# 3DOM-FBK/deep-image-matching

Hardware: NVIDIA H100
Metric: image-pairs/sec (SuperPoint+LightGlue, 1024x1024, 2048 kpts) (higher is better)
Workload: dtype f16 hi/lo split x3 MMA, f32 accumulate (fp32-class)

## Files before the change

### deep-image-matching_b200/csrc/attention.cuh

```cuda
#pragma once
#include "common.cuh"
#include "sm90.cuh"

namespace {

constexpr int kAttnBlk = 64;
constexpr int kAttnTile = 128;
constexpr int kAttnThreads = 9 * 32;

template <int HD, bool SPLIT>
struct AttnGeom {
  static constexpr int kPl = SPLIT ? 2 : 1;
  static constexpr int kAtoms = HD / 64;
  static constexpr int kAtomQ = kAttnTile * 128, kQB = kAtoms * kAtomQ;
  static constexpr int kAtomK = kAttnBlk * 128, kKB = kAtoms * kAtomK;
  static constexpr int kVB = HD * 128;
  static constexpr int kSmem = kPl * (kQB + 2 * (kKB + kVB)) + 256 + 1024;
};

template <int HD, bool SPLIT, class Out>
__device__ __forceinline__ void attn_tile(const CUtensorMap* tmQh, const CUtensorMap* tmQl, const CUtensorMap* tmKh,
                                          const CUtensorMap* tmKl, const CUtensorMap* tmVh, const CUtensorMap* tmVl, int qrow, int krow,
                                          int vrow, int nq, int nk, float scale, float lazy, const Out& out) {
  using namespace sm90;
  using G = AttnGeom<HD, SPLIT>;
  extern __shared__ uint8_t sm_attn_raw[];
  uint8_t* smem = sm_attn_raw + ((1024u - (smem_u32(sm_attn_raw) & 1023u)) & 1023u);
  uint8_t* sQ = smem;
  uint8_t* sK = sQ + G::kPl * G::kQB;
  uint8_t* sV = sK + 2 * G::kPl * G::kKB;
  uint64_t* bars = reinterpret_cast<uint64_t*>(sV + 2 * G::kPl * G::kVB);
  uint64_t *bQ = bars, *kFull = bars + 1, *kEmpty = bars + 3, *vFull = bars + 5, *vEmpty = bars + 7;
  const int tid = threadIdx.x, warp = tid >> 5, lane = tid & 31;
  if (tid == 0) {
    mbar_init(bQ, 1);
    for (int i = 0; i < 2; ++i) {
      mbar_init(&kFull[i], 1);
      mbar_init(&kEmpty[i], 8);
      mbar_init(&vFull[i], 1);
      mbar_init(&vEmpty[i], 8);
    }
    fence_barrier_init();
  }
  __syncthreads();
  const int nblk = (nk + kAttnBlk - 1) / kAttnBlk;

  if (warp == 8) {
    if (nblk > 0 && elect_one()) {
      mbar_expect_tx(bQ, G::kPl * G::kQB);
      for (int at = 0; at < G::kAtoms; ++at) {
        tma_load_2d(sQ + at * G::kAtomQ, tmQh, bQ, at * 64, qrow);
        if (SPLIT) tma_load_2d(sQ + G::kQB + at * G::kAtomQ, tmQl, bQ, at * 64, qrow);
      }
    }
    __syncwarp();
    for (int j = 0; j < nblk; ++j) {
      const int s = j & 1;
      const uint32_t ph = (j >> 1) & 1;
      mbar_wait(&kEmpty[s], ph ^ 1);
      if (elect_one()) {
        mbar_expect_tx(&kFull[s], G::kPl * G::kKB);
        for (int at = 0; at < G::kAtoms; ++at) {
          tma_load_2d(sK + s * G::kPl * G::kKB + at * G::kAtomK, tmKh, &kFull[s], at * 64, krow + j * kAttnBlk);
          if (SPLIT) tma_load_2d(sK + s * G::kPl * G::kKB + G::kKB + at * G::kAtomK, tmKl, &kFull[s], at * 64, krow + j * kAttnBlk);
        }
      }
      __syncwarp();
      mbar_wait(&vEmpty[s], ph ^ 1);
      if (elect_one()) {
        mbar_expect_tx(&vFull[s], G::kPl * G::kVB);
        tma_load_2d(sV + s * G::kPl * G::kVB, tmVh, &vFull[s], j * kAttnBlk, vrow);
        if (SPLIT) tma_load_2d(sV + s * G::kPl * G::kVB + G::kVB, tmVl, &vFull[s], j * kAttnBlk, vrow);
      }
      __syncwarp();
    }
    return;
  }
  const int wg = warp >> 2, w4 = warp & 3;
  const int r0 = 64 * wg + 16 * w4 + (lane >> 2);
  const uint32_t q_wg = smem_u32(sQ) + wg * 64 * 128;
  float o[HD / 2];
#pragma unroll
  for (int i = 0; i < HD / 2; ++i) o[i] = 0.f;
  float m_run[2] = {-INFINITY, -INFINITY}, l_run[2] = {0.f, 0.f};
  const float c2 = scale * 1.4426950408889634f;
  if (nblk > 0) mbar_wait(bQ, 0);
  for (int j = 0; j < nblk; ++j) {
    const int s = j & 1;
    const uint32_t ph = (j >> 1) & 1;
    float sc[kAttnBlk / 2];
    mbar_wait(&kFull[s], ph);
    {
      const uint32_t kb = smem_u32(sK + s * G::kPl * G::kKB);
      wgmma_fence();
#pragma unroll
      for (int kk = 0; kk < 4 * G::kAtoms; ++kk) {
        const uint64_t qh = sdesc_advance_k(make_sdesc_sw128(q_wg + (kk >> 2) * G::kAtomQ), kk & 3);
        const uint64_t kh = sdesc_advance_k(make_sdesc_sw128(kb + (kk >> 2) * G::kAtomK), kk & 3);
        Wgmma<kAttnBlk>::ss(sc, qh, kh, kk != 0);
        if (SPLIT) {
          const uint64_t ql = sdesc_advance_k(make_sdesc_sw128(q_wg + G::kQB + (kk >> 2) * G::kAtomQ), kk & 3);
          const uint64_t kl = sdesc_advance_k(make_sdesc_sw128(kb + G::kKB + (kk >> 2) * G::kAtomK), kk & 3);
          Wgmma<kAttnBlk>::ss(sc, qh, kl, 1);
          Wgmma<kAttnBlk>::ss(sc, ql, kh, 1);
        }
      }
      wgmma_commit();
      wgmma_wait<0>();
      wgmma_fence_regs(sc);
    }
    if (lane == 0) mbar_arrive(&kEmpty[s]);
    const int key0 = j * kAttnBlk + 2 * (lane & 3);
    if (j * kAttnBlk + kAttnBlk > nk) {
#pragma unroll
      for (int i = 0; i < kAttnBlk / 8; ++i)
#pragma unroll
        for (int e = 0; e < 4; ++e)
          if (key0 + 8 * i + (e & 1) >= nk) sc[4 * i + e] = -INFINITY;
    }
    float alpha[2], mc[2];
#pragma unroll
    for (int h = 0; h < 2; ++h) {
      float mx = sc[2 * h];
#pragma unroll
      for (int i = 0; i < kAttnBlk / 8; ++i) mx = fmaxf(mx, fmaxf(sc[4 * i + 2 * h], sc[4 * i + 2 * h + 1]));
      mx = fmaxf(mx, __shfl_xor_sync(0xffffffffu, mx, 1));
      mx = fmaxf(mx, __shfl_xor_sync(0xffffffffu, mx, 2));
      const float m_blk = fmaxf(m_run[h], mx);
      const bool grow = (m_blk - m_run[h]) * c2 > lazy;
      const float m_new = grow ? m_blk : m_run[h];
      alpha[h] = grow ? fast_exp2((m_run[h] - m_new) * c2) : 1.f;
      mc[h] = m_new * c2;
      m_run[h] = m_new;
    }
    float ps[2] = {0.f, 0.f};
#pragma unroll
    for (int i = 0; i < kAttnBlk / 8; ++i)
#pragma unroll
      for (int e = 0; e < 4; ++e) {
        sc[4 * i + e] = fast_exp2(fmaf(sc[4 * i + e], c2, -mc[e >> 1]));
        ps[e >> 1] += sc[4 * i + e];
      }
#pragma unroll
    for (int h = 0; h < 2; ++h) l_run[h] = l_run[h] * alpha[h] + ps[h];
#pragma unroll
    for (int i = 0; i < HD / 8; ++i) {
      o[4 * i] *= alpha[0], o[4 * i + 1] *= alpha[0];
      o[4 * i + 2] *= alpha[1], o[4 * i + 3] *= alpha[1];
    }
    uint32_t ph_[kAttnBlk / 4], pl_[kAttnBlk / 4];
#pragma unroll
    for (int c = 0; c < kAttnBlk / 4; ++c) {
      __half2 h2, l2;
      split2_f32(sc[2 * c], sc[2 * c + 1], h2, l2);
      ph_[c] = *reinterpret_cast<uint32_t*>(&h2);
      pl_[c] = *reinterpret_cast<uint32_t*>(&l2);
    }
    mbar_wait(&vFull[s], ph);
    {
      const uint32_t vb = smem_u32(sV + s * G::kPl * G::kVB);
      const uint64_t v_h = make_sdesc_sw128(vb), v_l = make_sdesc_sw128(vb + G::kVB);
      wgmma_fence();
#pragma unroll
      for (int kk = 0; kk < kAttnBlk / 16; ++kk) {
        const uint32_t ah[4] = {ph_[4 * kk], ph_[4 * kk + 1], ph_[4 * kk + 2], ph_[4 * kk + 3]};
        Wgmma<HD>::rs(o, ah, sdesc_advance_k(v_h, kk), 1);
        if (SPLIT) {
          const uint32_t al[4] = {pl_[4 * kk], pl_[4 * kk + 1], pl_[4 * kk + 2], pl_[4 * kk + 3]};
          Wgmma<HD>::rs(o, ah, sdesc_advance_k(v_l, kk), 1);
          Wgmma<HD>::rs(o, al, sdesc_advance_k(v_h, kk), 1);
        }
      }
      wgmma_commit();
      wgmma_wait<0>();
      wgmma_fence_regs(o);
    }
    if (lane == 0) mbar_arrive(&vEmpty[s]);
  }
  float inv[2];
#pragma unroll
  for (int h = 0; h < 2; ++h) {
    float l = l_run[h];
    l += __shfl_xor_sync(0xffffffffu, l, 1);
    l += __shfl_xor_sync(0xffffffffu, l, 2);
    inv[h] = nblk > 0 ? 1.f / l : 0.f;
  }
#pragma unroll
  for (int i = 0; i < HD / 8; ++i) {
    const int col = 8 * i + 2 * (lane & 3);
    if (r0 < nq) out(r0, col, o[4 * i] * inv[0], o[4 * i + 1] * inv[0]);
    if (r0 + 8 < nq) out(r0 + 8, col, o[4 * i + 2] * inv[1], o[4 * i + 3] * inv[1]);
  }
}

}
```

Measured before the change: 230.5.

## Software-pipeline attention: overlap next QK^T wgmma with current softmax and PV

Restructures the consumer loop so the S=QK^T wgmma for block j+1 is issued before the PV wgmma for block j, and the softmax of j+1 runs while PV is still in flight (wait<1>). The producer now prefetches K one block ahead of V to feed this ordering. It also skips the O rescale when no lane's running max grew. The cost is extra register pressure from keeping sc, ph_/pl_ and o live together, plus more complex barrier phase handling.

New measurement: 235.5 (median of 6 runs). 1.02x the previous value.

```diff
diff --git a/deep-image-matching_b200/csrc/attention.cuh b/deep-image-matching_b200/csrc/attention.cuh
--- a/deep-image-matching_b200/csrc/attention.cuh
+++ b/deep-image-matching_b200/csrc/attention.cuh
@@ -54,10 +54,9 @@
       }
     }
     __syncwarp();
-    for (int j = 0; j < nblk; ++j) {
+    const auto load_k = [&](int j) {
       const int s = j & 1;
-      const uint32_t ph = (j >> 1) & 1;
-      mbar_wait(&kEmpty[s], ph ^ 1);
+      mbar_wait(&kEmpty[s], ((j >> 1) & 1) ^ 1);
       if (elect_one()) {
         mbar_expect_tx(&kFull[s], G::kPl * G::kKB);
         for (int at = 0; at < G::kAtoms; ++at) {
@@ -66,6 +65,12 @@
         }
       }
       __syncwarp();
+    };
+    if (nblk > 0) load_k(0);
+    for (int j = 0; j < nblk; ++j) {
+      const int s = j & 1;
+      const uint32_t ph = (j >> 1) & 1;
+      if (j + 1 < nblk) load_k(j + 1);
       mbar_wait(&vEmpty[s], ph ^ 1);
       if (elect_one()) {
         mbar_expect_tx(&vFull[s], G::kPl * G::kVB);
@@ -78,38 +83,37 @@
   }
   const int wg = warp >> 2, w4 = warp & 3;
   const int r0 = 64 * wg + 16 * w4 + (lane >> 2);
-  const uint32_t q_wg = smem_u32(sQ) + wg * 64 * 128;
+  const uint32_t q_wg0 = smem_u32(sQ) + wg * 64 * 128;
   float o[HD / 2];
 #pragma unroll
   for (int i = 0; i < HD / 2; ++i) o[i] = 0.f;
   float m_run[2] = {-INFINITY, -INFINITY}, l_run[2] = {0.f, 0.f};
   const float c2 = scale * 1.4426950408889634f;
-  if (nblk > 0) mbar_wait(bQ, 0);
-  for (int j = 0; j < nblk; ++j) {
+  float sc[kAttnBlk / 2];
+  uint32_t ph_[kAttnBlk / 4], pl_[kAttnBlk / 4];
+  float alpha[2];
+  const auto issue_s = [&](int j) {
     const int s = j & 1;
-    const uint32_t ph = (j >> 1) & 1;
-    float sc[kAttnBlk / 2];
-    mbar_wait(&kFull[s], ph);
-    {
-      const uint32_t kb = smem_u32(sK + s * G::kPl * G::kKB);
-      wgmma_fence();
-#pragma unroll
-      for (int kk = 0; kk < 4 * G::kAtoms; ++kk) {
-        const uint64_t qh = sdesc_advance_k(make_sdesc_sw128(q_wg + (kk >> 2) * G::kAtomQ), kk & 3);
-        const uint64_t kh = sdesc_advance_k(make_sdesc_sw128(kb + (kk >> 2) * G::kAtomK), kk & 3);
-        Wgmma<kAttnBlk>::ss(sc, qh, kh, kk != 0);
-        if (SPLIT) {
-          const uint64_t ql = sdesc_advance_k(make_sdesc_sw128(q_wg + G::kQB + (kk >> 2) * G::kAtomQ), kk & 3);
-          const uint64_t kl = sdesc_advance_k(make_sdesc_sw128(kb + G::kKB + (kk >> 2) * G::kAtomK), kk & 3);
-          Wgmma<kAttnBlk>::ss(sc, qh, kl, 1);
-          Wgmma<kAttnBlk>::ss(sc, ql, kh, 1);
-        }
-      }
-      wgmma_commit();
-      wgmma_wait<0>();
-      wgmma_fence_regs(sc);
-    }
-    if (lane == 0) mbar_arrive(&kEmpty[s]);
+    mbar_wait(&kFull[s], (j >> 1) & 1);
+    const uint32_t kb = smem_u32(sK + s * G::kPl * G::kKB);
+    uint32_t q_wg;
+    asm volatile("mov.u32 %0, %1;" : "=r"(q_wg) : "r"(q_wg0));
+    wgmma_fence();
+#pragma unroll
+    for (int kk = 0; kk < 4 * G::kAtoms; ++kk) {
+      const uint64_t qh = sdesc_advance_k(make_sdesc_sw128(q_wg + (kk >> 2) * G::kAtomQ), kk & 3);
+      const uint64_t kh = sdesc_advance_k(make_sdesc_sw128(kb + (kk >> 2) * G::kAtomK), kk & 3);
+      Wgmma<kAttnBlk>::ss(sc, qh, kh, kk != 0);
+      if (SPLIT) {
+        const uint64_t ql = sdesc_advance_k(make_sdesc_sw128(q_wg + G::kQB + (kk >> 2) * G::kAtomQ), kk & 3);
+        const uint64_t kl = sdesc_advance_k(make_sdesc_sw128(kb + G::kKB + (kk >> 2) * G::kAtomK), kk & 3);
+        Wgmma<kAttnBlk>::ss(sc, qh, kl, 1);
+        Wgmma<kAttnBlk>::ss(sc, ql, kh, 1);
+      }
+    }
+    wgmma_commit();
+  };
+  const auto softmax = [&](int j) {
     const int key0 = j * kAttnBlk + 2 * (lane & 3);
     if (j * kAttnBlk + kAttnBlk > nk) {
 #pragma unroll
@@ -118,7 +122,8 @@
         for (int e = 0; e < 4; ++e)
           if (key0 + 8 * i + (e & 1) >= nk) sc[4 * i + e] = -INFINITY;
     }
-    float alpha[2], mc[2];
+    float mc[2];
+    bool grew = false;
 #pragma unroll
     for (int h = 0; h < 2; ++h) {
       float mx = sc[2 * h];
@@ -132,6 +137,7 @@
       alpha[h] = grow ? fast_exp2((m_run[h] - m_new) * c2) : 1.f;
       mc[h] = m_new * c2;
       m_run[h] = m_new;
+      grew |= grow;
     }
     float ps[2] = {0.f, 0.f};
 #pragma unroll
@@ -143,12 +149,16 @@
       }
 #pragma unroll
     for (int h = 0; h < 2; ++h) l_run[h] = l_run[h] * alpha[h] + ps[h];
-#pragma unroll
-    for (int i = 0; i < HD / 8; ++i) {
-      o[4 * i] *= alpha[0], o[4 * i + 1] *= alpha[0];
-      o[4 * i + 2] *= alpha[1], o[4 * i + 3] *= alpha[1];
-    }
-    uint32_t ph_[kAttnBlk / 4], pl_[kAttnBlk / 4];
+    return __any_sync(0xffffffffu, grew);
+  };
+  const auto rescale_split = [&](bool grew) {
+    if (grew) {
+#pragma unroll
+      for (int i = 0; i < HD / 8; ++i) {
+        o[4 * i] *= alpha[0], o[4 * i + 1] *= alpha[0];
+        o[4 * i + 2] *= alpha[1], o[4 * i + 3] *= alpha[1];
+      }
+    }
 #pragma unroll
     for (int c = 0; c < kAttnBlk / 4; ++c) {
       __half2 h2, l2;
@@ -156,26 +166,50 @@
       ph_[c] = *reinterpret_cast<uint32_t*>(&h2);
       pl_[c] = *reinterpret_cast<uint32_t*>(&l2);
     }
-    mbar_wait(&vFull[s], ph);
-    {
-      const uint32_t vb = smem_u32(sV + s * G::kPl * G::kVB);
-      const uint64_t v_h = make_sdesc_sw128(vb), v_l = make_sdesc_sw128(vb + G::kVB);
-      wgmma_fence();
-#pragma unroll
-      for (int kk = 0; kk < kAttnBlk / 16; ++kk) {
-        const uint32_t ah[4] = {ph_[4 * kk], ph_[4 * kk + 1], ph_[4 * kk + 2], ph_[4 * kk + 3]};
-        Wgmma<HD>::rs(o, ah, sdesc_advance_k(v_h, kk), 1);
-        if (SPLIT) {
-          const uint32_t al[4] = {pl_[4 * kk], pl_[4 * kk + 1], pl_[4 * kk + 2], pl_[4 * kk + 3]};
-          Wgmma<HD>::rs(o, ah, sdesc_advance_k(v_l, kk), 1);
-          Wgmma<HD>::rs(o, al, sdesc_advance_k(v_h, kk), 1);
-        }
-      }
-      wgmma_commit();
+  };
+  const auto issue_pv = [&](int j) {
+    const int s = j & 1;
+    mbar_wait(&vFull[s], (j >> 1) & 1);
+    const uint32_t vb = smem_u32(sV + s * G::kPl * G::kVB);
+    const uint64_t v_h = make_sdesc_sw128(vb), v_l = make_sdesc_sw128(vb + G::kVB);
+    wgmma_fence();
+#pragma unroll
+    for (int kk = 0; kk < kAttnBlk / 16; ++kk) {
+      const uint32_t ah[4] = {ph_[4 * kk], ph_[4 * kk + 1], ph_[4 * kk + 2], ph_[4 * kk + 3]};
+      Wgmma<HD>::rs(o, ah, sdesc_advance_k(v_h, kk), 1);
+      if (SPLIT) {
+        const uint32_t al[4] = {pl_[4 * kk], pl_[4 * kk + 1], pl_[4 * kk + 2], pl_[4 * kk + 3]};
+        Wgmma<HD>::rs(o, ah, sdesc_advance_k(v_l, kk), 1);
+        Wgmma<HD>::rs(o, al, sdesc_advance_k(v_h, kk), 1);
+      }
+    }
+    wgmma_commit();
+  };
+  if (nblk > 0) {
+    mbar_wait(bQ, 0);
+    issue_s(0);
+    wgmma_wait<0>();
+    wgmma_fence_regs(sc);
+    if (lane == 0) mbar_arrive(&kEmpty[0]);
+    bool grew = softmax(0);
+    for (int j = 0; j + 1 < nblk; ++j) {
       wgmma_wait<0>();
       wgmma_fence_regs(o);
-    }
-    if (lane == 0) mbar_arrive(&vEmpty[s]);
+      if (j > 0 && lane == 0) mbar_arrive(&vEmpty[(j - 1) & 1]);
+      rescale_split(grew);
+      issue_s(j + 1);
+      issue_pv(j);
+      wgmma_wait<1>();
+      wgmma_fence_regs(sc);
+      if (lane == 0) mbar_arrive(&kEmpty[(j + 1) & 1]);
+      grew = softmax(j + 1);
+    }
+    wgmma_wait<0>();
+    wgmma_fence_regs(o);
+    rescale_split(grew);
+    issue_pv(nblk - 1);
+    wgmma_wait<0>();
+    wgmma_fence_regs(o);
   }
   float inv[2];
 #pragma unroll
```
